# anyboby/Constrained-Model-Based-Policy-Optimization

Hardware: AMD Instinct MI355X
Metric: imagined env-steps/sec (ensemble rollout) + CPO update ms (higher is better)
Workload: dtype f32; 1 GPU; AntSafe-v2 imagined rollout: E=7 x (37->512->512->60) swish ensemble, 5 elites, 3+3 critics 128x128, tanh policy 128x128, B=100000 branches/GPU, maxroll 35 (34 steps), fixed-horizon mode, reset->sample*->finish_all_paths->get(); rollout_mode=schedule, branches_per_gpu=100000, branches_total=100000, horizon=34, task=AntSafe-v2

## Files before the change

### constrained-model-based-policy-optimization_amd/_lib.py

```python
import ctypes as C
import os

_HERE = os.path.dirname(os.path.abspath(__file__))
LIB_PATH = os.path.join(_HERE, "libcmbpo_hip.so")

ACT_SWISH, ACT_TANH = 0, 1
HEAD_PROB, HEAD_DETMEAN, HEAD_GAUSS_PI = 0, 1, 2
LOSS_DEFAULT, LOSS_NLL = 0, 1
ENS_FP32, ENS_SPLIT_BF16, ENS_SPLIT_F16 = 0, 1, 2
TASK_DEFAULT, TASK_HCS, TASK_ANTSAFE = 0, 1, 2
TASK_LEARNED_COST = 0x100
TASK_USER_BASE, TASK_USER_SLOTS = 16, 64
RULE_MAX_CLAUSES = 16
RULE_HEALTHY, RULE_FATAL, RULE_COST = 0, 1, 2
RULE_SRC_NEXT_OBS, RULE_SRC_OBS, RULE_SRC_ACT = 0, 1, 2
RULE_ABS, RULE_LO_STRICT, RULE_HI_STRICT, RULE_ANY = 1, 2, 4, 8

TASK_IDS = {
    "default": TASK_DEFAULT,
    "HalfCheetah-v2": TASK_DEFAULT,
    "HalfCheetahSafe-v2": TASK_HCS,
    "AntSafe-v2": TASK_ANTSAFE,
}

_p = C.c_void_p
_i = C.c_int
_sz = C.c_size_t

SIGNATURES = {
    "cmbpo_last_error": (C.c_char_p, []),
    "cmbpo_version": (_i, []),
    "cmbpo_set_ens_matrix_path": (_i, [_i]),
    "cmbpo_get_ens_matrix_path": (_i, []),
    "cmbpo_set_ens_f16_min_rows": (_i, [_i]),
    "cmbpo_set_ens_f16_row_tiles": (_i, [_i]),
    "cmbpo_mlp_create": (_i, [C.POINTER(_p), _i, _i, _i, _i, _i, _i]),
    "cmbpo_mlp_destroy": (None, [_p]),
    "cmbpo_mlp_load": (_i, [_p] * 13),
    "cmbpo_mlp_load_policy_flat": (_i, [_p, _p, _p]),
    "cmbpo_ens_forward": (_i, [_p, _p, _i, _p, _i, _p, _p, _i, _i, _p, _p, _p]),
    "cmbpo_ens_predict_mean": (_i, [_p, _p, _i, _p, _p, _i, _p, _p]),
    "cmbpo_critic_pair_supported": (_i, [_p, _p]),
    "cmbpo_critic_pair_predict": (_i, [_p, _p, _p, _i, _p, _p, _i, _p, _p, _p]),
    "cmbpo_critic_pair_predict_var": (_i, [_p, _p, _p, _i, _p, _p, _i, C.c_float, C.c_float, _p, _p, _p, _p, _p]),
    "cmbpo_policy_forward": (_i, [_p, _p, _i, _p, _p, _p, _i, _p, _p, _p, _p, _p]),
    "cmbpo_fakeenv_post": (_i, [_i, _i, _i, _i, _p, _p, _i, _p, _p, _p, _p, _p, _i,
                                _p, _p, _p, _p, _p, _p, _p, _p]),
    "cmbpo_fakeenv_post_noise": (_i, [_i, _i, _i, _i, _p, _p, _i, _p, _p, _p, _p, _p, _i,
                                      _p, _p, _p, _p, _p, _p, _p, _p, _p]),
    "cmbpo_fakeenv_post_disagreement": (_i, [_i, _i, _i, _i, _p, _p, _i, _p, _p, _p, _p, _p, _i,
                                             _p, _p, _p, _p, _p, _p, _p, _p, C.c_float, C.c_float, _p, _p, _p]),
}



class RuleClauseStruct(C.Structure):
    _fields_ = [(n, C.c_int32) for n in ("role", "src", "col0", "n_cols", "flags")] + \
               [(n, C.c_float) for n in ("scale", "lo", "hi")]


class TaskRulesStruct(C.Structure):
    _fields_ = [(n, C.c_int32) for n in ("n_clauses", "require_finite", "cost_on_term", "reserved")] + \
               [("clause", RuleClauseStruct * RULE_MAX_CLAUSES)]


SIGNATURES.update({
    "cmbpo_task_rules_register": (_i, [C.POINTER(TaskRulesStruct), C.POINTER(C.c_int)]),
    "cmbpo_task_rules_get": (_i, [_i, C.POINTER(TaskRulesStruct)]),
# ... 283 lines not shown
```

### constrained-model-based-policy-optimization_amd/csrc/ens_h3.hip

```cpp
#include "common.h"
#include "ens_mlp_internal.h"
#include "f16_split.h"

#include <type_traits>

namespace {

constexpr int kThreadsH = 512;
constexpr int kWavesH = 8;
constexpr int HIDH = 512;

template <int RT>
struct Geo {
  static constexpr int ROWS = 32 * RT;
  static constexpr int NTC = 8 / RT;
  static constexpr int CK = 32 * NTC;
  static constexpr int NCH = HIDH / CK;
  static constexpr int SLC = CK / 32;
  static constexpr int CSTR = CK + 8;
  static constexpr int TPR = kThreadsH / ROWS;
  static constexpr int KPT = 64 / TPR;
  static constexpr int DH = RT == 4 ? 2 : 4;
  static constexpr int NPH = (2 * SLC) % DH == 0 ? 1 : DH;
  static constexpr int CBUF_BYTES = 2 * ROWS * CSTR * 2;
// ... 94 lines not shown
    float v = 0.0f;
    if ((n >> 5) < src_tiles && (k >> 3) < kg) v = sp[pack_index_tile(n >> 5, r, k, kg)];
    _Float16 q1, q2;
    split_h(v * scale, q1, q2);
    p1[j] = q1; p2[j] = q2;
  }
  f16x8 *d = dst + (size_t)e * dst_stride + IMAGE_INDEX(tile, slabs, s, 2, 0) + lane;
  d[0] = p1; d[kImageLanes] = p2;
}

template <int I, int N, class F>
__device__ __forceinline__ void static_for(F &&f) {
  if constexpr (I < N) {
    f(std::integral_constant<int, I>{});
    static_for<I + 1, N>(f);
  }
}


constexpr int kPieces = 24, kReqEarly = 5;
__host__ __device__ constexpr int piece_at(int slot, int i) {
  if (i % 2 != 0) return -1;
  const int k = i / 2;
  if (slot == 0) return k % 3 == 0 ? k / 3 : -1;
  if (slot == 1) return k == 0 ? 4 : (k == 2 ? 5 : (k == 4 ? 6 : -1));
  if (slot == 3) return k == 4 ? 13 : -1;
  if (slot == 4) return k == 1 ? 7 : -1;
  if (slot == 5) return k == 4 ? 20 : (k >= 6 && k < 10 ? 2 + k : -1);
  if (slot == 6) return k == 0 ? 12 : (k == 1 ? 14 : (k == 3 ? 15 : (k == 5 ? 16 : (k >= 7 && k <= 9 ? 10 + k : (k == 10 ? 21 : -1)))));
  if (slot == 7) return k < 2 ? 22 + k : -1;
  return -1;
}

struct H3Args {
  MlpKernelArgs m;
  const f16x8 *w0, *w1, *w2;
  size_t w0_stride, w1_stride, w2_stride;
  const float *stats;
  int item0;
};

template <int S0, int OTP, int RT>
__global__ __launch_bounds__(kThreadsH, 2) void ens_h3_kernel(const H3Args a) {
  using G = Geo<RT>;
  constexpr int ROWSH = G::ROWS, NTC = G::NTC, CK = G::CK, NCH = G::NCH, SLC = G::SLC, CSTR = G::CSTR, TPR = G::TPR,
                KPT = G::KPT, DH = G::DH, NPH = G::NPH, CBUF_BYTES = G::CBUF_BYTES;
  constexpr int XSTR = 16 * S0 + 8;
  constexpr int NPASS = OTP / 2;
  constexpr int NUNIT = RT * NPASS;
  constexpr int O_PAD = 32 * OTP;
  constexpr int W0P = NTC * S0 * 2;
  constexpr bool AHEAD = stage_ahead(S0, RT);
  const MlpKernelArgs &p = a.m;
  extern __shared__ f32x4 smem4[];
  char *smem = reinterpret_cast<char *>(smem4);
  _Float16 *cbuf = reinterpret_cast<_Float16 *>(smem);
  _Float16 *ximg = reinterpret_cast<_Float16 *>(smem + off_ximg(S0, RT));
  f16x8 *w0buf = reinterpret_cast<f16x8 *>(smem + off_ximg(S0, RT) + ximg_bytes(S0, RT));
  constexpr bool PB2 = !AHEAD;
  f32x4 *pbuf = reinterpret_cast<f32x4 *>(smem);
  float *stg = reinterpret_cast<float *>(smem + (PB2 ? 2 : 1) * PBUF_BYTES);
  float *cst = reinterpret_cast<float *>(smem + off_const(S0, RT));
  struct Cst { float *bias0, *bias1, *hc_a, *hc_c; int *rowidx; float *r_inv0, *r_t1, *r_inv1, *r_t2, *r_inv2; };
  auto cst_of = [&](int par) {
    Cst c;
    c.bias0 = cst + (AHEAD ? par : 0) * ITEM_FLOATS; c.bias1 = c.bias0 + HIDH; c.hc_a = c.bias0 + 2 * HIDH; c.hc_c = c.hc_a + 128;
    c.rowidx = reinterpret_cast<int *>(c.hc_c + 128);
    c.r_inv0 = c.hc_c + 256; c.r_t1 = c.r_inv0 + 128; c.r_inv1 = c.r_t1 + 128; c.r_t2 = c.r_inv1 + 128; c.r_inv2 = c.r_t2 + 128;
    return c;
  };
  float *in_mu_l = cst + (AHEAD ? 2 : 1) * ITEM_FLOATS, *in_sig_l = in_mu_l + 64;

  const int n_rows = p.n_rows_dev ? *p.n_rows_dev : p.n_rows;
  const int out = p.out_dim;
  if (threadIdx.x < 64) {
    const int k = threadIdx.x;
    in_mu_l[k] = (p.in_mu && k < p.in_dim) ? p.in_mu[k] : 0.0f;
    in_sig_l[k] = (p.in_mu && k < p.in_dim) ? 1.0f / p.in_sig[k] : 1.0f;
  }
  __syncthreads();

  auto next_alive = [&](int it) {
    while (it < p.n_items) {
      const int e2 = it / p.tiles;
      if ((it - e2 * p.tiles) * ROWSH < n_rows) break;
      it += gridDim.x;
    }
    return it;
  };
  int rr_pre = -1;
  auto fetch_row = [&](int it, int tid) {
    const int xb = tid / TPR;
    const int e2 = it / p.tiles;
    const int rr = (it - e2 * p.tiles) * ROWSH + xb;
    const bool ok = it < p.n_items && rr < n_rows;
    int v = ok ? rr : 0;
    if (p.row_idx) v = p.row_idx[v];
    rr_pre = ok ? v : -1;
  };

  constexpr int W0R = G::W0_LDS ? (2 * W0P + kWavesH - 1) / kWavesH : 1;
  constexpr int GQ = KPT / 4;
  struct StageRegs {
    float x[KPT];
    float b0, b1, b2, hs, hm, hl;
    float st[7];
    f16x8 w0r[W0R];
    float m, t0, t1, t2;
    unsigned q1[KPT / 2], q2[KPT / 2];
  };
  auto stage_piece = [&](auto KC, auto FRONTC, StageRegs &s, const int es, const Cst &c, const int tid, const int it_next) {
    constexpr int K = decltype(KC)::value;
    constexpr bool FRONT = decltype(FRONTC)::value;
    const int xb = tid / TPR, xc = tid % TPR;
    if constexpr (K < 4) {
      const int rr = rr_pre >= 0 ? rr_pre : 0;
      const float *orow = p.obs + (size_t)rr * p.obs_dim;
      const float *arow = p.act_dim > 0 ? p.act + (size_t)rr * p.act_dim - p.obs_dim : orow;
#pragma unroll
      for (int u = GQ * K; u < GQ * K + GQ; ++u) {
        const int k = KPT * xc + u;
        const bool in_obs = k < p.obs_dim, in_act = !in_obs & (k < p.in_dim);
        const float *base = in_act ? arow : orow;
        const int off = (in_obs | in_act) ? k : 0;
        s.x[u] = base[off];
      }
    } else if constexpr (K == 4) {
      s.b0 = p.b0[(size_t)es * HIDH + tid];
      s.b1 = p.b1[(size_t)es * HIDH + tid];
      const int ob = p.o_tiles * 32;
      s.b2 = p.b2[(size_t)es * ob + (tid < ob ? tid : 0)];
    } else if constexpr (K == 5) {
      s.hs = 1.0f; s.hm = 0.0f; s.hl = 0.0f;
      if (p.out_mu) {
        const int ia = tid < out ? tid : out - 1, il = tid < out ? 0 : (tid < 2 * out ? tid - out : out - 1);
        s.hs = p.out_sig[ia]; s.hm = p.out_mu[ia]; s.hl = p.out_lsig2[il];
      }
      const float *st = a.stats + (size_t)es * NSTAT;
      s.st[0] = st[0]; s.st[1] = st[1]; s.st[2] = st[2]; s.st[3] = st[4]; s.st[4] = st[5]; s.st[5] = st[6]; s.st[6] = st[8];
    } else if constexpr (K == 6 || K == 13 || K == 20 || K == 22) {
      if constexpr (G::W0_LDS) {
        const int lane = tid & 63, wave = __builtin_amdgcn_readfirstlane(tid >> 6);
        const f16x8 *w0s = a.w0 + (size_t)es * a.w0_stride;
        auto get = [&](f16x8 &x, int u) { const int j = wave + kWavesH * u; x = w0s[(size_t)(j < 2 * W0P ? j : 0) * 64 + lane]; };
        auto put = [&](const f16x8 &x, int u) { const int j = wave + kWavesH * u; if (j < 2 * W0P) w0buf[(size_t)j * 64 + lane] = x; };
        if constexpr (FRONT) {
#pragma unroll
          for (int u = 0; u < W0R; ++u) {
            if constexpr (K == 6) get(s.w0r[u], u);
            if constexpr (K == 22) put(s.w0r[u], u);
          }
        } else {
          constexpr int u = K == 6 ? 0 : (K == 13 ? 1 : (K == 20 ? 2 : 3));
          static_assert(W0R <= 3, "ens_h3: rounds of the W0 chunks");
          if constexpr (u >= 1 && u <= W0R) put(s.w0r[0], u - 1);
          if constexpr (u < W0R) get(s.w0r[0], u);
        }
      }
    } else if constexpr (K == 7) {
      c.bias0[tid] = s.b0 * kLog2e;
      c.bias1[tid] = s.b1 * kLog2e;
      if (tid < O_PAD) {
        const bool is_mean = tid < out, is_var = !is_mean & (tid < 2 * out);
        float A = is_var ? 1.0f : 0.0f, Bc = is_var ? s.hl : 0.0f;
        A = is_mean ? s.hs : A; Bc = is_mean ? s.hm : Bc;
        c.hc_a[tid] = A;
        c.hc_c[tid] = A * s.b2 + Bc;
      }
    } else if constexpr (K < 12) {
      if constexpr (K == 8) s.m = 0.0f;
#pragma unroll
      for (int u = GQ * (K - 8); u < GQ * (K - 8) + GQ; ++u) {
        const int k = KPT * xc + u;
        float x = (s.x[u] - in_mu_l[k & 63]) * in_sig_l[k & 63];
        const bool keep = (k < p.in_dim) & (rr_pre >= 0);
        x = keep ? x : 0.0f;
        s.x[u] = x;
        s.m = fmaxf(s.m, fabsf(x));
        asm volatile("" : "+v"(s.x[u]));
      }
      asm volatile("" : "+v"(s.m));
    } else if constexpr (K == 12) {
#pragma unroll
      for (int o = 1; o < TPR; o <<= 1) s.m = fmaxf(s.m, __shfl_xor(s.m, o, 64));
      s.t0 = pow2_lift(s.m);
      asm volatile("" : "+v"(s.m), "+v"(s.t0));
    } else if constexpr (K == 14) {
      if (xc == 0) {
        const float bound1 = (s.st[1] * s.m + s.st[2]) * 1.001f, t1 = pow2_lift(bound1);
        const float bound2 = (s.st[4] * bound1 + s.st[5]) * 1.001f, t2 = pow2_lift(bound2);
        c.rowidx[xb] = rr_pre;
        c.r_inv0[xb] = 1.0f / (s.st[0] * s.t0);
        c.r_t1[xb] = t1;
        c.r_t2[xb] = t2;
        s.t1 = t1; s.t2 = t2;
      }
    } else if constexpr (K == 15) {
      if (xc == 0) {
        c.r_inv1[xb] = 1.0f / (s.st[3] * s.t1);
        c.r_inv2[xb] = 1.0f / (s.st[6] * s.t2);
      }
    } else if constexpr (K < 20) {
#pragma unroll
      for (int u = GQ * (K - 16); u < GQ * (K - 16) + GQ; ++u) {
        _Float16 h1, h2;
        split_h(s.x[u] * s.t0, h1, h2);
        if (u % 2 == 0) { s.q1[u / 2] = __builtin_bit_cast(unsigned short, h1); s.q2[u / 2] = __builtin_bit_cast(unsigned short, h2); }
        else {
          s.q1[u / 2] |= (unsigned)__builtin_bit_cast(unsigned short, h1) << 16;
          s.q2[u / 2] |= (unsigned)__builtin_bit_cast(unsigned short, h2) << 16;
          asm volatile("" : "+v"(s.q1[u / 2]), "+v"(s.q2[u / 2]));
        }
      }
    } else if constexpr (K == 21) {
      if (KPT * xc < 16 * S0) {
        _Float16 *d1 = ximg + (size_t)xb * XSTR + KPT * xc, *d2 = d1 + (size_t)ROWSH * XSTR;
        if constexpr (KPT >= 8) {
#pragma unroll
          for (int v = 0; v < KPT / 8; ++v) {
            u32x4 w1, w2;
#pragma unroll
// ... 156 lines not shown
          constexpr int i = decltype(IC)::value;
          const int pos = 2 * slot + i / 12;
          const int sl = pos / VT, v = pos % VT;
          const int u = (i % 12) / 3, term = i % 3;
          const int hl = 2 * sl + (u >> 1);
          f16x8(&Ah)[2][2] = A[(PH * 2 * SLC + hl) % DH];
          if (i % 12 == 0) {
            if (pos + 1 < 16) read_b(Bt[(pos + 1) & 1], img, (pos + 1) % VT, (pos + 1) / VT);
            if (i == 0) __builtin_amdgcn_sched_barrier(0);
          }
          f32x4 &ac = acc[u][v];
          const f16x8 &b1 = Bt[pos & 1][0], &b2 = Bt[pos & 1][1];
          if (term == 0) ac = __builtin_amdgcn_mfma_f32_16x16x32_f16(Ah[u & 1][1], b1, ac, 0, 0, 0);
          else if (term == 1) ac = __builtin_amdgcn_mfma_f32_16x16x32_f16(Ah[u & 1][0], b2, ac, 0, 0, 0);
          else ac = __builtin_amdgcn_mfma_f32_16x16x32_f16(Ah[u & 1][0], b1, ac, 0, 0, 0);
          if (v == VT - 1 && (i % 12 == 5 || i % 12 == 11) && !(LAST && hl + DH >= 2 * SLC))
            load_h(Ah, c * 2 * SLC + hl + DH);
          if (!LAST && slot < S0 && i == 11) {
            mm3(d, l0.a1, l0.a2, l0.b1, l0.b2);
            if (slot + 1 < S0) l0_read(l0, c + 1, slot + 1);
          }
          if (!LAST && slot >= 4 && i % 2 == 0) {
            const int q = slot - 4, k = i / 2;
            if (k == 0) epi_stage<0, true>(es, d, q, inv0_l, bv, t1_l);
            if (k == 2) epi_stage<2, true>(es, d, q, inv0_l, bv, t1_l);
            if (k == 3) epi_stage<3, true>(es, d, q, inv0_l, bv, t1_l);
            if (k == 4) epi_stage<4, true>(es, d, q, inv0_l, bv, t1_l);
            if (k == 5) epi_stage<5, true>(es, d, q, inv0_l, bv, t1_l);
            if (k == 6) epi_stage<6, true>(es, d, q, inv0_l, bv, t1_l);
            if (k == 8) epi_stage<8, true>(es, d, q, inv0_l, bv, t1_l);
            if (k == 9) epi_stage<9, true>(es, d, q, inv0_l, bv, t1_l);
            if (k == 10) l0_store(es, c + 1, q);
          }
          if constexpr (STG && piece_at(slot, i) >= 0)
            if (have_next) stage_piece(std::integral_constant<int, (piece_at(slot, i) >= 0 ? piece_at(slot, i) : 0)>{}, std::false_type{}, sa, e_nxt, cn, tid_s, nxt2);
          __builtin_amdgcn_sched_barrier(0);
        });
      });
      if constexpr (STG) {
        static_for<0, 24>([&](auto IC) {
          constexpr int pc = piece_at(8, decltype(IC)::value);
          if constexpr (pc >= 0)
            if (have_next) stage_piece(std::integral_constant<int, (pc >= 0 ? pc : 0)>{}, std::false_type{}, sa, e_nxt, cn, tid_s, nxt2);
        });
      }
      H3_STAMP(4);
      if constexpr (G::W0_LDS && !LAST) {
        if (stage_w0) {
          const int j = W0P > kWavesH ? wave + kWavesH : wave;
          if (j < W0P) w0buf[((size_t)(c & 1) * W0P + j) * 64 + lane] = wst;
        }
      }
      lds_barrier();
      H3_STAMP(5);
    };
    {
      constexpr int NREG = NCH - 1, NFULL = NREG / NPH * NPH;
#pragma unroll 1
      for (int c0 = 0; c0 < NFULL; c0 += NPH)
        static_for<0, NPH>([&](auto P) { step(std::false_type{}, c0 + decltype(P)::value, P); });
      static_for<0, NREG - NFULL>([&](auto P) { step(std::false_type{}, NFULL + decltype(P)::value, P); });
      step(std::true_type{}, NREG, std::integral_constant<int, NREG % NPH>{});
    }
    if constexpr (!AHEAD) {
      if (nxt < p.n_items) static_for<0, kReqEarly>([&](auto P) { stage_piece(P, std::true_type{}, sr, e_nxt, cc, tid, 0); });
    }
    H3_STAMP(6);

    const f16x8 *w2w = a.w2 + (size_t)e * a.w2_stride + lane;
    auto reduce_unit = [&](int u) {
      const int rt = u / NPASS, pass = u % NPASS;
      const int tt = wave >> 2, q = wave & 3;
      const f32x4 *pp = pbuf + ((size_t)(PB2 ? u & 1 : 0) * 64 + (size_t)tt * 4 + q) * 64 + lane;
      f32x4 v = pp[0];
// ... 190 lines not shown
      m->d_h3 = nullptr;
      cmbpo_set_error("ens_h3: hipMalloc of the f16 weight images failed");
      return CMBPO_ENOMEM;
    }
    m->h3_version = ~0ul;
  }
  if (m->h3_version == m->pack_version) return CMBPO_OK;
  float *stats = reinterpret_cast<float *>(reinterpret_cast<char *>(m->d_h3) + m->h3_stats_off * 16);
  cmbpo_internal_f16_stats(m, stats, s);
  for (int l = 0; l < 3; ++l)
    cmbpo_internal_f16_pack(m, l, reinterpret_cast<f16x8 *>(m->d_h3) + m->h3_off[l], m->h3_stride[l], tiles[l], slabs[l],
                            l == 0 ? 0 : l + 1, stats, s);
  CMBPO_HIP_CHECK(hipGetLastError());
  m->h3_version = m->pack_version;
  return CMBPO_OK;
}

void cmbpo_internal_f16_stats(const cmbpo_mlp *m, float *stats, hipStream_t s) {
  hipLaunchKernelGGL(h3_stats_kernel, dim3(m->ensemble, 3), dim3(kThreadsH), 0, s, m->d_blob, m->off_wp0, m->off_wp1, m->off_wp2,
                     m->off_b0, m->off_b1, m->off_b2, m->in_pad / 8, m->o_tiles, m->hidden, stats);
}
void cmbpo_internal_f16_pack(const cmbpo_mlp *m, int layer, void *dst, size_t dst_stride, int n_tiles, int slabs, int perm,
                             const float *stats, hipStream_t s) {
  const long total = (long)(IMAGE_UNITS(n_tiles, slabs, 1) * m->ensemble);
  hipLaunchKernelGGL(h3_pack_kernel, dim3((unsigned)((total + 255) / 256)), dim3(256), 0, s, m->pack(layer), m->pack_floats(layer),
                     m->pack_kg(layer), m->pack_tiles(layer), reinterpret_cast<f16x8 *>(dst), dst_stride, n_tiles, slabs, m->ensemble,
                     stats, layer, perm);
}

static int g_h3_rt = 0;
extern "C" int cmbpo_set_ens_f16_row_tiles(int rt) {
  CMBPO_REQUIRE(rt == 0 || rt == 1 || rt == 2 || rt == 4, "cmbpo_set_ens_f16_row_tiles: 0 (by row count), 1, 2 or 4");
  g_h3_rt = rt;
  return CMBPO_OK;
}

bool cmbpo_internal_h3_eligible(const cmbpo_mlp *m) {
  return m->head == CMBPO_HEAD_PROB && m->hidden == 512 && m->act == CMBPO_ACT_SWISH && m->o_tiles <= 4 && m->in_pad <= 64 &&
         2 * m->out_dim == m->o_width;
}

int cmbpo_internal_launch_h3(cmbpo_mlp *m, MlpKernelArgs &a, hipStream_t s) {
  if (m->h3_s0 == 0) {
    const int s0 = (m->in_pad + 15) / 16;
    m->h3_s0 = s0 < 2 ? 2 : s0;
    m->h3_otp = m->o_tiles <= 2 ? 2 : 4;
  }
  if (int rc = ensure_h3(m, s)) return rc;
  H3Args k{};
  k.m = a;
  const f16x8 *base = reinterpret_cast<const f16x8 *>(m->d_h3);
  k.w0 = base + m->h3_off[0]; k.w1 = base + m->h3_off[1]; k.w2 = base + m->h3_off[2];
  k.w0_stride = m->h3_stride[0]; k.w1_stride = m->h3_stride[1]; k.w2_stride = m->h3_stride[2];
  k.stats = reinterpret_cast<const float *>(reinterpret_cast<const char *>(m->d_h3) + m->h3_stats_off * 16);
  const int n_cu = cmbpo_cu_count();
  const int E = m->ensemble;
  constexpr int kSplitGap = 40;
  int RT = g_h3_rt, RT_tail = 0, full = 0, tail_start = 0;
  if (RT == 0) {
    const int first_two[3] = {220, 310, 550}, steady_two[3] = {175, 300, 540};
    const int first_four[3] = {255, 360, 720}, steady_four[3] = {198, 343, 705};
    const int *first = m->h3_otp > 2 ? first_four : first_two, *steady = m->h3_otp > 2 ? steady_four : steady_two;
    const int rts[3] = {1, 2, 4};
    auto cost_of = [&](int i, long rounds) -> long { return rounds <= 0 ? 0 : first[i] + (rounds - 1) * steady[i]; };
    long best = -1;
    for (int i = 0; i < 3; ++i) {
      const long cost = cost_of(i, cmbpo_ceil_div(cmbpo_ceil_div(a.n_rows, 32 * rts[i]) * E, n_cu));
      if (best < 0 || cost <= best) { best = cost; RT = rts[i]; }
    }
    for (int i = 1; i < 3; ++i) {
      const int tiles_m = cmbpo_ceil_div(a.n_rows, 32 * rts[i]), n_m = tiles_m * E;
      const int fl = n_m / n_cu * n_cu, left = n_m - fl;
      if (fl == 0 || left == 0) continue;
      const int e0 = fl / tiles_m, t0 = fl - e0 * tiles_m;
      for (int j = 0; j < i; ++j) {
        const int tiles_t = cmbpo_ceil_div(a.n_rows, 32 * rts[j]);
        const int start = e0 * tiles_t + (rts[i] / rts[j]) * t0, n_tail = tiles_t * E - start;
        const long cost = cost_of(i, fl / n_cu) + cost_of(j, cmbpo_ceil_div(n_tail, n_cu)) + kSplitGap;
        if (cost < best) { best = cost; RT = rts[i]; RT_tail = rts[j]; full = fl; tail_start = start; }
      }
    }
  }
  const int S0 = m->h3_s0, OTP = m->h3_otp;
  auto launch = [&](int rt, int item0, int end) -> int {
    const int tiles = cmbpo_ceil_div(a.n_rows, 32 * rt);
    k.m.tiles = tiles;
    k.m.n_items = end < 0 ? tiles * E : end;
    k.item0 = item0;
    const size_t lds = (size_t)lds_bytes(S0, rt);
    CMBPO_REQUIRE(lds <= 160 * 1024, "ens_h3: LDS budget exceeded (%zu B)", lds);
    const int n_here = k.m.n_items - item0;
    const int grid = n_here < n_cu ? n_here : n_cu;
#define CMBPO_H3_CASE(S0_, OTP_, RT_)                                                                                  \
  if (S0 == S0_ && OTP == OTP_ && rt == RT_) {                                                                         \
    if (int rc = cmbpo_grant_lds(ens_h3_kernel<S0_, OTP_, RT_>, lds)) return rc;                                      \
    hipLaunchKernelGGL((ens_h3_kernel<S0_, OTP_, RT_>), dim3(grid), dim3(kThreadsH), lds, s, k);                      \
  }
#define CMBPO_H3_CASES(RT_)                                                                                            \
  CMBPO_H3_CASE(2, 2, RT_) CMBPO_H3_CASE(3, 2, RT_) CMBPO_H3_CASE(4, 2, RT_)                                           \
  CMBPO_H3_CASE(2, 4, RT_) CMBPO_H3_CASE(3, 4, RT_) CMBPO_H3_CASE(4, 4, RT_)
    CMBPO_H3_CASES(4) CMBPO_H3_CASES(2) CMBPO_H3_CASES(1)
#undef CMBPO_H3_CASES
#undef CMBPO_H3_CASE
    CMBPO_HIP_CHECK(hipGetLastError());
    return CMBPO_OK;
  };
  if (RT_tail) {
    if (int rc = launch(RT, 0, full)) return rc;
    return launch(RT_tail, tail_start, -1);
  }
  return launch(RT, 0, -1);
}
```

### constrained-model-based-policy-optimization_amd/csrc/ens_mlp.hip

```cpp
#include "common.h"
#include "ens_mlp_internal.h"
#include "mfma_tile.h"

#include <math.h>
#include <string.h>
#include <vector>

#ifdef CMBPO_STAMPS
static unsigned long long *g_stamps = nullptr;
extern "C" void cmbpo_debug_set_stamps(unsigned long long *p) { g_stamps = p; }
#define STAMP(k)                                                                                   \
  do {                                                                                             \
    if (p.stamps && threadIdx.x == 0)                                                              \
      p.stamps[(size_t)stamp_item * 12 + (k)] =                                  \
          ((k) >= 8 ? __builtin_amdgcn_s_memrealtime() : __builtin_amdgcn_s_memtime());                 \
  } while (0)
#else
#define STAMP(k)
#endif

namespace {

constexpr int kThreads = 256;
constexpr int kWaves = 4;
// ... 461 lines not shown
  m->out_dim = (head == CMBPO_HEAD_PROB) ? out_width / 2 : out_width;
  m->act = activation; m->head = head; m->loaded = false;
  m->has_in_scaler = m->has_out_scaler = false;

  const int E = ensemble, H = hidden;
  size_t off = 0;
  auto take = [&](size_t n) { size_t o = off; off += (n + 3) / 4 * 4; return o; };
  m->off_wp0 = take(E * m->pack_floats(0));
  m->off_wp1 = take(E * m->pack_floats(1));
  m->off_wp2 = take(E * m->pack_floats(2));
  m->off_b0 = take((size_t)E * H);
  m->off_b1 = take((size_t)E * H);
  m->off_b2 = take((size_t)E * m->o_tiles * 32);
  m->off_in_mu = take(in_dim); m->off_in_var = take(in_dim);
  m->off_out_mu = take(m->out_dim); m->off_out_var = take(m->out_dim); m->off_out_lsig2 = take(m->out_dim);
  m->off_log_std = take(m->out_dim);
  m->blob_floats = off;
  m->d_blob = nullptr;
  hipError_t err = hipMalloc(reinterpret_cast<void **>(&m->d_blob), off * sizeof(float));
  if (err != hipSuccess) {
    cmbpo_set_error("cmbpo_mlp_create: hipMalloc(%zu) failed: %s", off * sizeof(float), hipGetErrorString(err));
    delete m;
    return CMBPO_ENOMEM;
  }
  *out = m;
  return CMBPO_OK;
}

extern "C" void cmbpo_mlp_destroy(cmbpo_mlp_t *m) {
  if (!m) return;
  if (m->d_blob) (void)hipFree(m->d_blob);
  if (m->d_split) (void)hipFree(m->d_split);
  if (m->d_h3) (void)hipFree(m->d_h3);
  delete m;
}

extern "C" int cmbpo_mlp_load(cmbpo_mlp_t *m, const float *h_w0, const float *h_b0,
                              const float *h_w1, const float *h_b1, const float *h_w2,
                              const float *h_b2, const float *h_in_mu, const float *h_in_var,
                              const float *h_out_mu, const float *h_out_var,
                              const float *h_log_std, void *stream) {
  CMBPO_REQUIRE(m != nullptr, "cmbpo_mlp_load: handle is NULL");
  CMBPO_REQUIRE(h_w0 && h_b0 && h_w1 && h_b1 && h_w2 && h_b2, "cmbpo_mlp_load: weight pointer is NULL");
  CMBPO_REQUIRE((h_in_mu == nullptr) == (h_in_var == nullptr), "cmbpo_mlp_load: in scaler needs both mu and var");
  CMBPO_REQUIRE((h_out_mu == nullptr) == (h_out_var == nullptr), "cmbpo_mlp_load: out scaler needs both mu and var");
  if (m->head == CMBPO_HEAD_GAUSS_PI)
    CMBPO_REQUIRE(h_log_std != nullptr, "cmbpo_mlp_load: policy head needs log_std");
  const int E = m->ensemble, H = m->hidden, I = m->in_dim, O = m->o_width;
  m->h_blob.assign(m->blob_floats, 0.0f);
  float *hb = m->h_blob.data();
  for (int e = 0; e < E; ++e) {
    pack_weights(h_w0 + (size_t)e * I * H, I, H, m->in_pad, H / 32, hb + m->off_wp0 + e * m->pack_floats(0));
    pack_weights(h_w1 + (size_t)e * H * H, H, H, H, H / 32, hb + m->off_wp1 + e * m->pack_floats(1));
    pack_weights(h_w2 + (size_t)e * H * O, H, O, H, m->o_tiles, hb + m->off_wp2 + e * m->pack_floats(2));
    memcpy(hb + m->off_b0 + (size_t)e * H, h_b0 + (size_t)e * H, H * sizeof(float));
    memcpy(hb + m->off_b1 + (size_t)e * H, h_b1 + (size_t)e * H, H * sizeof(float));
    memcpy(hb + m->off_b2 + (size_t)e * m->o_tiles * 32, h_b2 + (size_t)e * O, O * sizeof(float));
  }
  m->has_in_scaler = h_in_mu != nullptr;
  m->has_out_scaler = h_out_mu != nullptr;
  if (h_in_mu) {
    memcpy(hb + m->off_in_mu, h_in_mu, I * sizeof(float));
    for (int k = 0; k < I; ++k) hb[m->off_in_var + k] = fmaxf(sqrtf(h_in_var[k]), 1e-2f);
  }
  if (h_out_mu) {
    memcpy(hb + m->off_out_mu, h_out_mu, m->out_dim * sizeof(float));
// ... 217 lines not shown
```

### constrained-model-based-policy-optimization_amd/csrc/ens_mlp_internal.h

```cpp
#pragma once
#include "common.h"
#include "pack_layout.h"

#include <vector>

#define CMBPO_HEAD_TRAIN 3

struct MlpKernelArgs {
  const f32x4 *wp0, *wp1, *wp2;
  size_t wp0_stride, wp1_stride, wp2_stride;
  const float *b0, *b1, *b2;
  const float *in_mu, *in_sig;
  const float *out_mu, *out_sig, *out_lsig2;
  const float *log_std;
  int ensemble, e_chunk;
  int in_dim, in_pad;
  int o_width, o_tiles, out_dim;
  const float *obs;
  int obs_dim;
  const float *act;
  int act_dim;
  const float *eps;
  const int32_t *row_idx;
  const int32_t *n_rows_dev;
// ... 1 lines not shown
  int ld_rows;
  float *out0;
  float *out1;
  float *out2;
  float *out3;
  unsigned long long *stamps;
  int stagger_sleeps;
  int tiles, n_items, n_cu;
  int row_idx_stride;
  float *tr_x;
  float *tr_h1, *tr_g1;
  float *tr_h2, *tr_g2;
  const float *tr_targets;
  int tr_tdim;
  double *tr_loss_part;
  float *tr_opmax;
};

struct cmbpo_mlp {
  int ensemble, in_dim, in_pad, hidden, o_width, o_tiles, out_dim, act, head;
  bool loaded, has_in_scaler, has_out_scaler;
  float *d_blob;
  size_t blob_floats;
  size_t off_wp0, off_wp1, off_wp2, off_b0, off_b1, off_b2;
  size_t off_in_mu, off_in_var, off_out_mu, off_out_var, off_out_lsig2, off_log_std;
  std::vector<float> h_blob;
  void *d_split = nullptr;
  unsigned long pack_version = 0, split_version = ~0ul;
  size_t sp_off[3] = {0, 0, 0}, sp_stride[3] = {0, 0, 0};
  void *d_h3 = nullptr;
  unsigned long h3_version = ~0ul;
  size_t h3_off[3] = {0, 0, 0}, h3_stride[3] = {0, 0, 0}, h3_stats_off = 0;
  int h3_s0 = 0, h3_otp = 0;
  int pack_tiles(int l) const { return l == 2 ? o_tiles : hidden / 32; }
  int pack_kg(int l) const { return (l == 0 ? in_pad : hidden) / 8; }
  size_t pack_floats(int l) const { return ::pack_floats(pack_tiles(l), pack_kg(l)); }
  float *pack(int l) const { return d_blob + (l == 0 ? off_wp0 : l == 1 ? off_wp1 : off_wp2); }
  const float *in_mu() const { return has_in_scaler ? d_blob + off_in_mu : nullptr; }
  const float *in_sig() const { return has_in_scaler ? d_blob + off_in_var : nullptr; }
  const float *out_mu() const { return has_out_scaler ? d_blob + off_out_mu : nullptr; }
  const float *out_sig() const { return has_out_scaler ? d_blob + off_out_var : nullptr; }
  const float *out_lsig2() const { return has_out_scaler ? d_blob + off_out_lsig2 : nullptr; }
};

int cmbpo_internal_launch_mlp(cmbpo_mlp *m, MlpKernelArgs &a, hipStream_t s, int head_override);
int cmbpo_internal_launch_split(cmbpo_mlp *m, MlpKernelArgs &a, hipStream_t s);
bool cmbpo_internal_h3_eligible(const cmbpo_mlp *m);
int cmbpo_internal_launch_h3(cmbpo_mlp *m, MlpKernelArgs &a, hipStream_t s);
bool cmbpo_internal_policy_f16_eligible(const cmbpo_mlp *m);
int cmbpo_internal_launch_policy_f16(cmbpo_mlp *m, const MlpKernelArgs &a, hipStream_t s);
int cmbpo_internal_policy_f16_args(cmbpo_mlp *m, void *pf_args, int *s0_out, hipStream_t s);
constexpr int kCriticBigMin = 24576;
bool cmbpo_internal_critic_pair_can_ride(const cmbpo_mlp *v, const cmbpo_mlp *vc, const cmbpo_mlp *policy);
struct CmbpoStoreVec {
  const float *src[4];
  float *dst[4];
  int dim[4];
  const uint8_t *fin_code;
  size_t col_off;
};
struct CmbpoValueDis {
  float kappa_v, kappa_vc;
  float *v_var, *vc_var;
};
int cmbpo_internal_critic_pair_ride(cmbpo_mlp *v, cmbpo_mlp *vc, const float *d_obs, int obs_dim, const int32_t *d_row_idx,
                                    const int32_t *d_n_rows, int n_rows, float *d_v, float *d_vc, cmbpo_mlp *policy,
// ... 4 lines not shown
```

### include/cmbpo_hip.h

```cpp
#ifndef CMBPO_HIP_H
#define CMBPO_HIP_H

#include <stddef.h>
#include <stdint.h>

#ifdef __cplusplus
extern "C" {
#endif

#define CMBPO_OK 0
#define CMBPO_EINVAL (-1)
#define CMBPO_EHIP (-2)
#define CMBPO_ENOMEM (-3)
#define CMBPO_ESTATE (-4)

#define CMBPO_ACT_SWISH 0
#define CMBPO_ACT_TANH 1

#define CMBPO_HEAD_PROB 0
#define CMBPO_HEAD_DETMEAN 1
#define CMBPO_HEAD_GAUSS_PI 2

#define CMBPO_TASK_DEFAULT 0
#define CMBPO_TASK_HCS 1
// ... 8 lines not shown
#define CMBPO_RULE_COST 2
#define CMBPO_RULE_SRC_NEXT_OBS 0
#define CMBPO_RULE_SRC_OBS 1
#define CMBPO_RULE_SRC_ACT 2
#define CMBPO_RULE_ABS 1
#define CMBPO_RULE_LO_STRICT 2
#define CMBPO_RULE_HI_STRICT 4
#define CMBPO_RULE_ANY 8

typedef struct cmbpo_rule_clause {
  int32_t role, src, col0, n_cols, flags;
  float scale, lo, hi;
} cmbpo_rule_clause_t;

typedef struct cmbpo_task_rules {
  int32_t n_clauses, require_finite, cost_on_term, reserved;
  cmbpo_rule_clause_t clause[CMBPO_RULE_MAX_CLAUSES];
} cmbpo_task_rules_t;

int cmbpo_task_rules_register(const cmbpo_task_rules_t *rules, int *out_task);
int cmbpo_task_rules_get(int task, cmbpo_task_rules_t *out);
int cmbpo_task_rules_count(void);

const char *cmbpo_last_error(void);
int cmbpo_version(void);

#define CMBPO_ENS_FP32 0
#define CMBPO_ENS_SPLIT_BF16 1
#define CMBPO_ENS_SPLIT_F16 2
int cmbpo_set_ens_matrix_path(int path);
int cmbpo_get_ens_matrix_path(void);
int cmbpo_set_ens_f16_min_rows(int rows);
int cmbpo_set_ens_f16_row_tiles(int rt);

typedef struct cmbpo_mlp cmbpo_mlp_t;

int cmbpo_mlp_create(cmbpo_mlp_t **out, int ensemble, int in_dim, int hidden,
                     int out_width, int activation, int head);
void cmbpo_mlp_destroy(cmbpo_mlp_t *m);

int cmbpo_mlp_load(cmbpo_mlp_t *m, const float *h_w0, const float *h_b0,
                   const float *h_w1, const float *h_b1, const float *h_w2,
                   const float *h_b2, const float *h_in_mu,
                   const float *h_in_var, const float *h_out_mu,
                   const float *h_out_var, const float *h_log_std,
                   void *stream);

int cmbpo_mlp_load_policy_flat(cmbpo_mlp_t *m, const float *d_flat, void *stream);

int cmbpo_ens_forward(cmbpo_mlp_t *m, const float *d_obs, int obs_dim,
                      const float *d_act, int act_dim, const int32_t *d_row_idx,
                      const int32_t *d_n_rows, int n_rows, int ld_rows,
                      float *d_mean, float *d_var, void *stream);

int cmbpo_ens_predict_mean(cmbpo_mlp_t *m, const float *d_obs, int obs_dim,
                           const int32_t *d_row_idx, const int32_t *d_n_rows,
                           int n_rows, float *d_out, void *stream);

int cmbpo_critic_pair_supported(const cmbpo_mlp_t *v, const cmbpo_mlp_t *vc);
int cmbpo_critic_pair_predict(cmbpo_mlp_t *v, cmbpo_mlp_t *vc, const float *d_obs, int obs_dim,
                              const int32_t *d_row_idx, const int32_t *d_n_rows, int n_rows,
                              float *d_v, float *d_vc, void *stream);
int cmbpo_critic_pair_predict_var(cmbpo_mlp_t *v, cmbpo_mlp_t *vc, const float *d_obs, int obs_dim,
                                  const int32_t *d_row_idx, const int32_t *d_n_rows, int n_rows,
                                  float kappa_v, float kappa_vc, float *d_v, float *d_vc,
                                  float *d_v_var, float *d_vc_var, void *stream);
// ... 382 lines not shown
```

Measured before the change: 75.63 million imagined env-steps/s.

## Precompute normalized split-f16 input image once and DMA it into LDS per tile

Adds a pre-pass kernel that normalizes each 128-row tile of obs/act inputs once, splits it into hi/lo f16 halves and stores a tile image plus the per-row max in global memory. The main ensemble kernel, in the new image instances, then pulls the whole tile image straight into LDS with global_load_lds and skips the per-ensemble-member gather, normalize and split staging pieces, using a reshuffled staging schedule. This removes input work repeated for each of the 7 ensemble members. In exchange it adds an extra kernel launch, a device buffer, and a global round trip for the image.

```diff
diff --git a/constrained-model-based-policy-optimization_amd/_lib.py b/constrained-model-based-policy-optimization_amd/_lib.py
--- a/constrained-model-based-policy-optimization_amd/_lib.py
+++ b/constrained-model-based-policy-optimization_amd/_lib.py
@@ -34,6 +34,7 @@
     "cmbpo_get_ens_matrix_path": (_i, []),
     "cmbpo_set_ens_f16_min_rows": (_i, [_i]),
     "cmbpo_set_ens_f16_row_tiles": (_i, [_i]),
+    "cmbpo_set_ens_f16_image_min_rows": (_i, [_i]),
     "cmbpo_mlp_create": (_i, [C.POINTER(_p), _i, _i, _i, _i, _i, _i]),
     "cmbpo_mlp_destroy": (None, [_p]),
     "cmbpo_mlp_load": (_i, [_p] * 13),
diff --git a/constrained-model-based-policy-optimization_amd/csrc/ens_h3.hip b/constrained-model-based-policy-optimization_amd/csrc/ens_h3.hip
--- a/constrained-model-based-policy-optimization_amd/csrc/ens_h3.hip
+++ b/constrained-model-based-policy-optimization_amd/csrc/ens_h3.hip
@@ -150,15 +150,87 @@
   return -1;
 }
 
+__host__ __device__ constexpr int piece_at_img(int slot, int i) {
+  if (i % 2 != 0) return -1;
+  const int k = i / 2;
+  if (slot == 1) return k == 0 ? 4 : (k == 2 ? 5 : (k == 4 ? 6 : -1));
+  if (slot == 3) return k == 4 ? 13 : -1;
+  if (slot == 4) return k == 1 ? 7 : (k == 3 ? 2 : (k == 5 ? 0 : (k == 7 ? 1 : -1)));
+  if (slot == 5) return k == 4 ? 20 : -1;
+  if (slot == 6) return k == 1 ? 14 : (k == 3 ? 15 : -1);
+  if (slot == 7) return k < 2 ? 22 + k : -1;
+  return -1;
+}
+__host__ __device__ constexpr int piece_of(bool img, int slot, int i) { return img ? piece_at_img(slot, i) : piece_at(slot, i); }
+
 struct H3Args {
   MlpKernelArgs m;
   const f16x8 *w0, *w1, *w2;
   size_t w0_stride, w1_stride, w2_stride;
   const float *stats;
   int item0;
+  const char *ximg;
 };
 
-template <int S0, int OTP, int RT>
+__host__ __device__ constexpr int ximg_block_bytes(int S0) { return ximg_bytes(S0, 4) + 128 * 4; }
+template <int S0>
+__global__ __launch_bounds__(kThreadsH) void h3_ximage_kernel(const MlpKernelArgs p, char *img) {
+  static_assert(S0 < 4 && ximg_block_bytes(S0) % 512 == 0, "h3_ximage_kernel: pad halves are written by the thread behind the row's last element");
+  constexpr int XSTR = 16 * S0 + 8, TPR = Geo<4>::TPR, KPT = Geo<4>::KPT;
+  const int n_rows = p.n_rows_dev ? *p.n_rows_dev : p.n_rows;
+  const int tid = threadIdx.x, xb = tid / TPR, xc = tid % TPR;
+  __shared__ float mu_l[64], isig_l[64];
+  if (tid < 64) {
+    mu_l[tid] = (p.in_mu && tid < p.in_dim) ? p.in_mu[tid] : 0.0f;
+    isig_l[tid] = (p.in_mu && tid < p.in_dim) ? 1.0f / p.in_sig[tid] : 1.0f;
+  }
+  __syncthreads();
+  const int rr = blockIdx.x * 128 + xb;
+  const bool ok = rr < n_rows;
+  int v = ok ? rr : 0;
+  if (p.row_idx) v = p.row_idx[v];
+  const float *orow = p.obs + (size_t)v * p.obs_dim;
+  const float *arow = p.act_dim > 0 ? p.act + (size_t)v * p.act_dim - p.obs_dim : orow;
+  float x[KPT];
+  float m = 0.0f;
+#pragma unroll
+  for (int u = 0; u < KPT; ++u) {
+    const int k = KPT * xc + u;
+    const bool in_obs = k < p.obs_dim, in_act = !in_obs & (k < p.in_dim);
+    const float *base = in_act ? arow : orow;
+    const float raw = base[(in_obs | in_act) ? k : 0];
+    float xv = (raw - mu_l[k]) * isig_l[k];
+    xv = ((k < p.in_dim) & ok) ? xv : 0.0f;
+    x[u] = xv;
+    m = fmaxf(m, fabsf(xv));
+  }
+#pragma unroll
+  for (int o = 1; o < TPR; o <<= 1) m = fmaxf(m, __shfl_xor(m, o, 64));
+  const float t0 = pow2_lift(m);
+  char *blk = img + (size_t)blockIdx.x * ximg_block_bytes(S0);
+  _Float16 *d1 = reinterpret_cast<_Float16 *>(blk) + (size_t)xb * XSTR + KPT * xc, *d2 = d1 + (size_t)128 * XSTR;
+  if (KPT * xc < 16 * S0) {
+#pragma unroll
+    for (int w = 0; w < KPT / 8; ++w) {
+      f16x8 h1, h2;
+#pragma unroll
+      for (int j = 0; j < 8; ++j) {
+        _Float16 a, b;
+        split_h(x[8 * w + j] * t0, a, b);
+        h1[j] = a; h2[j] = b;
+      }
+      reinterpret_cast<f16x8 *>(d1)[w] = h1; reinterpret_cast<f16x8 *>(d2)[w] = h2;
+    }
+  } else if (KPT * xc == 16 * S0) {
+    f16x8 z;
+#pragma unroll
+    for (int j = 0; j < 8; ++j) z[j] = (_Float16)0.0f;
+    *reinterpret_cast<f16x8 *>(d1) = z; *reinterpret_cast<f16x8 *>(d2) = z;
+  }
+  if (xc == 0) reinterpret_cast<float *>(blk + ximg_bytes(S0, 4))[xb] = m;
+}
+
+template <int S0, int OTP, int RT, bool IMG = false>
 __global__ __launch_bounds__(kThreadsH, 2) void ens_h3_kernel(const H3Args a) {
   using G = Geo<RT>;
   constexpr int ROWSH = G::ROWS, NTC = G::NTC, CK = G::CK, NCH = G::NCH, SLC = G::SLC, CSTR = G::CSTR, TPR = G::TPR,
@@ -169,6 +241,9 @@
   constexpr int O_PAD = 32 * OTP;
   constexpr int W0P = NTC * S0 * 2;
   constexpr bool AHEAD = stage_ahead(S0, RT);
+  static_assert(!IMG || (AHEAD && RT == 4), "ens_h3: the image instances are the stage-ahead ones at 128 rows");
+  constexpr int NXP = ximg_bytes(S0, RT) / 1024;
+  static_assert(!IMG || ximg_bytes(S0, RT) % 1024 == 0, "ens_h3: the x image in whole LDS-DMA pieces");
   const MlpKernelArgs &p = a.m;
   extern __shared__ f32x4 smem4[];
   char *smem = reinterpret_cast<char *>(smem4);
@@ -191,7 +266,7 @@
 
   const int n_rows = p.n_rows_dev ? *p.n_rows_dev : p.n_rows;
   const int out = p.out_dim;
-  if (threadIdx.x < 64) {
+  if (!IMG && threadIdx.x < 64) {
     const int k = threadIdx.x;
     in_mu_l[k] = (p.in_mu && k < p.in_dim) ? p.in_mu[k] : 0.0f;
     in_sig_l[k] = (p.in_mu && k < p.in_dim) ? 1.0f / p.in_sig[k] : 1.0f;
@@ -207,9 +282,11 @@
     return it;
   };
   int rr_pre = -1;
+  int tile_pre = 0;
   auto fetch_row = [&](int it, int tid) {
     const int xb = tid / TPR;
     const int e2 = it / p.tiles;
+    if constexpr (IMG) tile_pre = it < p.n_items ? it - e2 * p.tiles : 0;
     const int rr = (it - e2 * p.tiles) * ROWSH + xb;
     const bool ok = it < p.n_items && rr < n_rows;
     int v = ok ? rr : 0;
@@ -231,7 +308,27 @@
     constexpr int K = decltype(KC)::value;
     constexpr bool FRONT = decltype(FRONTC)::value;
     const int xb = tid / TPR, xc = tid % TPR;
-    if constexpr (K < 4) {
+    if constexpr (IMG && (K < 4 || (K >= 8 && K <= 12) || (K >= 16 && K <= 19) || K == 21)) {
+      const char *blk = a.ximg + (size_t)tile_pre * ximg_block_bytes(S0);
+      if constexpr (K < 2) {
+        const int lane = tid & 63, wave = __builtin_amdgcn_readfirstlane(tid >> 6);
+        const unsigned lds_x = (unsigned)(unsigned long)(__attribute__((address_space(3))) char *)(smem + off_ximg(S0, RT));
+#pragma unroll
+        for (int u = 2 * K; u < 2 * K + 2; ++u) {
+          const int j = wave + kWavesH * u;
+          if (kWavesH * u < NXP && j < NXP) {
+            const char *g = blk + (size_t)j * 1024 + lane * 16;
+            const unsigned d = __builtin_amdgcn_readfirstlane(lds_x + j * 1024);
+            unsigned keep;
+            asm volatile("s_mov_b32 %0, m0\n\ts_mov_b32 m0, %2\n\ts_nop 0\n\tglobal_load_lds_dwordx4 %1, off\n\ts_mov_b32 m0, %0"
+                         : "=&s"(keep) : "v"(g), "s"(d) : "memory");
+          }
+        }
+        static_assert(NXP <= 4 * kWavesH, "ens_h3: pieces 0 / 1 request the whole x image");
+      } else if constexpr (K == 2) {
+        s.m = reinterpret_cast<const float *>(blk + ximg_bytes(S0, RT))[xb];
+      }
+    } else if constexpr (K < 4) {
       const int rr = rr_pre >= 0 ? rr_pre : 0;
       const float *orow = p.obs + (size_t)rr * p.obs_dim;
       const float *arow = p.act_dim > 0 ? p.act + (size_t)rr * p.act_dim - p.obs_dim : orow;
@@ -275,6 +372,7 @@
           if constexpr (u < W0R) get(s.w0r[0], u);
         }
       }
+      if constexpr (IMG && K == 22) asm volatile("s_waitcnt vmcnt(0)" ::: "memory");
     } else if constexpr (K == 7) {
       c.bias0[tid] = s.b0 * kLog2e;
       c.bias1[tid] = s.b1 * kLog2e;
@@ -305,6 +403,7 @@
       asm volatile("" : "+v"(s.m), "+v"(s.t0));
     } else if constexpr (K == 14) {
       if (xc == 0) {
+        if constexpr (IMG) s.t0 = pow2_lift(s.m);
         const float bound1 = (s.st[1] * s.m + s.st[2]) * 1.001f, t1 = pow2_lift(bound1);
         const float bound2 = (s.st[4] * bound1 + s.st[5]) * 1.001f, t2 = pow2_lift(bound2);
         c.rowidx[xb] = rr_pre;
@@ -527,14 +626,14 @@
             if (k == 9) epi_stage<9, true>(es, d, q, inv0_l, bv, t1_l);
             if (k == 10) l0_store(es, c + 1, q);
           }
-          if constexpr (STG && piece_at(slot, i) >= 0)
-            if (have_next) stage_piece(std::integral_constant<int, (piece_at(slot, i) >= 0 ? piece_at(slot, i) : 0)>{}, std::false_type{}, sa, e_nxt, cn, tid_s, nxt2);
+          if constexpr (STG && piece_of(IMG, slot, i) >= 0)
+            if (have_next) stage_piece(std::integral_constant<int, (piece_of(IMG, slot, i) >= 0 ? piece_of(IMG, slot, i) : 0)>{}, std::false_type{}, sa, e_nxt, cn, tid_s, nxt2);
           __builtin_amdgcn_sched_barrier(0);
         });
       });
       if constexpr (STG) {
         static_for<0, 24>([&](auto IC) {
-          constexpr int pc = piece_at(8, decltype(IC)::value);
+          constexpr int pc = piece_of(IMG, 8, decltype(IC)::value);
           if constexpr (pc >= 0)
             if (have_next) stage_piece(std::integral_constant<int, (pc >= 0 ? pc : 0)>{}, std::false_type{}, sa, e_nxt, cn, tid_s, nxt2);
         });
@@ -791,6 +890,29 @@
 extern "C" int cmbpo_set_ens_f16_row_tiles(int rt) {
   CMBPO_REQUIRE(rt == 0 || rt == 1 || rt == 2 || rt == 4, "cmbpo_set_ens_f16_row_tiles: 0 (by row count), 1, 2 or 4");
   g_h3_rt = rt;
+  return CMBPO_OK;
+}
+
+static int g_h3_img_min_rows = 0;
+extern "C" int cmbpo_set_ens_f16_image_min_rows(int rows) {
+  g_h3_img_min_rows = rows;
+  return CMBPO_OK;
+}
+
+static int ensure_ximg(cmbpo_mlp *m, int n_rows, int ld_rows, size_t block_bytes) {
+  const size_t need = (size_t)cmbpo_ceil_div(n_rows, 128);
+  if (m->d_ximg != nullptr && m->ximg_tiles >= need && m->ximg_block == block_bytes) return CMBPO_OK;
+  if (m->d_ximg) (void)hipFree(m->d_ximg);
+  m->d_ximg = nullptr; m->ximg_tiles = 0;
+  const size_t slots = ld_rows > 0 ? (size_t)cmbpo_ceil_div(ld_rows, 128) : 0;
+  const size_t tiles = need > slots ? need : slots;
+  if (hipMalloc(&m->d_ximg, tiles * block_bytes) != hipSuccess) {
+    (void)hipGetLastError();
+    m->d_ximg = nullptr;
+    cmbpo_set_error("ens_h3: hipMalloc of the input image (%zu B) failed", tiles * block_bytes);
+    return CMBPO_ENOMEM;
+  }
+  m->ximg_tiles = tiles; m->ximg_block = block_bytes;
   return CMBPO_OK;
 }
 
@@ -841,7 +963,7 @@
     }
   }
   const int S0 = m->h3_s0, OTP = m->h3_otp;
-  auto launch = [&](int rt, int item0, int end) -> int {
+  auto launch = [&](int rt, int item0, int end, bool main) -> int {
     const int tiles = cmbpo_ceil_div(a.n_rows, 32 * rt);
     k.m.tiles = tiles;
     k.m.n_items = end < 0 ? tiles * E : end;
@@ -850,23 +972,36 @@
     CMBPO_REQUIRE(lds <= 160 * 1024, "ens_h3: LDS budget exceeded (%zu B)", lds);
     const int n_here = k.m.n_items - item0;
     const int grid = n_here < n_cu ? n_here : n_cu;
-#define CMBPO_H3_CASE(S0_, OTP_, RT_)                                                                                  \
-  if (S0 == S0_ && OTP == OTP_ && rt == RT_) {                                                                         \
-    if (int rc = cmbpo_grant_lds(ens_h3_kernel<S0_, OTP_, RT_>, lds)) return rc;                                      \
-    hipLaunchKernelGGL((ens_h3_kernel<S0_, OTP_, RT_>), dim3(grid), dim3(kThreadsH), lds, s, k);                      \
-  }
+    const bool img = main && rt == 4 && stage_ahead(S0, 4) && g_h3_img_min_rows >= 0 &&
+                     (g_h3_img_min_rows == 0 ? n_here >= 2 * n_cu : a.n_rows >= g_h3_img_min_rows);
+    k.ximg = nullptr;
+    if (img) {
+      if (int rc = ensure_ximg(m, a.n_rows, a.ld_rows, (size_t)ximg_block_bytes(S0))) return rc;
+      k.ximg = reinterpret_cast<const char *>(m->d_ximg);
+      if (S0 == 2) hipLaunchKernelGGL(h3_ximage_kernel<2>, dim3(tiles), dim3(kThreadsH), 0, s, k.m, reinterpret_cast<char *>(m->d_ximg));
+      else hipLaunchKernelGGL(h3_ximage_kernel<3>, dim3(tiles), dim3(kThreadsH), 0, s, k.m, reinterpret_cast<char *>(m->d_ximg));
+      CMBPO_HIP_CHECK(hipGetLastError());
+    }
+#define CMBPO_H3_CASE_I(S0_, OTP_, RT_, IMG_)                                                                          \
+  if (S0 == S0_ && OTP == OTP_ && rt == RT_ && img == IMG_) {                                                          \
+    if (int rc = cmbpo_grant_lds(ens_h3_kernel<S0_, OTP_, RT_, IMG_>, lds)) return rc;                                \
+    hipLaunchKernelGGL((ens_h3_kernel<S0_, OTP_, RT_, IMG_>), dim3(grid), dim3(kThreadsH), lds, s, k);                \
+  }
+#define CMBPO_H3_CASE(S0_, OTP_, RT_) CMBPO_H3_CASE_I(S0_, OTP_, RT_, false)
 #define CMBPO_H3_CASES(RT_)                                                                                            \
   CMBPO_H3_CASE(2, 2, RT_) CMBPO_H3_CASE(3, 2, RT_) CMBPO_H3_CASE(4, 2, RT_)                                           \
   CMBPO_H3_CASE(2, 4, RT_) CMBPO_H3_CASE(3, 4, RT_) CMBPO_H3_CASE(4, 4, RT_)
     CMBPO_H3_CASES(4) CMBPO_H3_CASES(2) CMBPO_H3_CASES(1)
+    CMBPO_H3_CASE_I(2, 2, 4, true) CMBPO_H3_CASE_I(3, 2, 4, true) CMBPO_H3_CASE_I(2, 4, 4, true) CMBPO_H3_CASE_I(3, 4, 4, true)
 #undef CMBPO_H3_CASES
 #undef CMBPO_H3_CASE
+#undef CMBPO_H3_CASE_I
     CMBPO_HIP_CHECK(hipGetLastError());
     return CMBPO_OK;
   };
   if (RT_tail) {
-    if (int rc = launch(RT, 0, full)) return rc;
-    return launch(RT_tail, tail_start, -1);
-  }
-  return launch(RT, 0, -1);
-}
+    if (int rc = launch(RT, 0, full, true)) return rc;
+    return launch(RT_tail, tail_start, -1, false);
+  }
+  return launch(RT, 0, -1, true);
+}
diff --git a/constrained-model-based-policy-optimization_amd/csrc/ens_mlp.hip b/constrained-model-based-policy-optimization_amd/csrc/ens_mlp.hip
--- a/constrained-model-based-policy-optimization_amd/csrc/ens_mlp.hip
+++ b/constrained-model-based-policy-optimization_amd/csrc/ens_mlp.hip
@@ -517,6 +517,7 @@
   if (m->d_blob) (void)hipFree(m->d_blob);
   if (m->d_split) (void)hipFree(m->d_split);
   if (m->d_h3) (void)hipFree(m->d_h3);
+  if (m->d_ximg) (void)hipFree(m->d_ximg);
   delete m;
 }
 
diff --git a/constrained-model-based-policy-optimization_amd/csrc/ens_mlp_internal.h b/constrained-model-based-policy-optimization_amd/csrc/ens_mlp_internal.h
--- a/constrained-model-based-policy-optimization_amd/csrc/ens_mlp_internal.h
+++ b/constrained-model-based-policy-optimization_amd/csrc/ens_mlp_internal.h
@@ -57,6 +57,8 @@
   unsigned long h3_version = ~0ul;
   size_t h3_off[3] = {0, 0, 0}, h3_stride[3] = {0, 0, 0}, h3_stats_off = 0;
   int h3_s0 = 0, h3_otp = 0;
+  void *d_ximg = nullptr;
+  size_t ximg_tiles = 0, ximg_block = 0;
   int pack_tiles(int l) const { return l == 2 ? o_tiles : hidden / 32; }
   int pack_kg(int l) const { return (l == 0 ? in_pad : hidden) / 8; }
   size_t pack_floats(int l) const { return ::pack_floats(pack_tiles(l), pack_kg(l)); }
diff --git a/include/cmbpo_hip.h b/include/cmbpo_hip.h
--- a/include/cmbpo_hip.h
+++ b/include/cmbpo_hip.h
@@ -64,6 +64,7 @@
 int cmbpo_get_ens_matrix_path(void);
 int cmbpo_set_ens_f16_min_rows(int rows);
 int cmbpo_set_ens_f16_row_tiles(int rt);
+int cmbpo_set_ens_f16_image_min_rows(int rows);
 
 typedef struct cmbpo_mlp cmbpo_mlp_t;
 
```

Result: faster. 78.02 million imagined env-steps/s, median of 6 (+3.2%).
